# schmeing/ReSeq

Hardware: AMD Instinct MI355X
Metric: simulated read-pairs/sec (2x150 bp) (higher is better)
Workload: dtype f64

## Files before the change

### reseq_amd/csrc/rsq_kernels.h

```cpp
#pragma once
#include "rsq_core.h"
#include "rsq_variants.h"

namespace rsq {

struct Chain {
    uint32_t kind;
    uint32_t id;
    uint32_t seg;
    uint32_t len;
    uint32_t c1, c2;
    uint32_t first_chunk;
    uint32_t initial_dom;
    uint16_t *out;
    uint32_t chunk_lo = 0, in_state = 0;
};

struct ChainAcc {
    const uint64_t *words;
    uint32_t kind, len;
    uint64_t word_off;
    const uint8_t *codes;
    RSQ_HD uint32_t operator()(uint32_t pos) const {
        if (kind == 0) return ref_base(words, word_off, pos);
// ... 959 lines not shown
template <>
struct WordPtr<RSQ_LDS char *> {
    using type = RSQ_LDS uint32_t *;
};
#endif
template <class P>
struct WordSinkT : TextOps<WordSinkT<P>> {
    P p;
    uint64_t acc;
    uint32_t pending, lead, n;
    RSQ_HD explicit WordSinkT(P dst) : p(dst), acc(0), pending(0), lead((4u - ((uint32_t)(uintptr_t)dst & 3u)) & 3u), n(0) {}
    RSQ_HD void push(uint32_t bytes, uint32_t count) {
        acc |= (uint64_t)bytes << (8u * pending);
        pending += count;
        n += count;
        while (lead && pending) {
            *p = (char)(acc & 0xFFu);
            p += 1;
            acc >>= 8;
            --pending;
            --lead;
        }
        if (!lead && pending >= 4u) {
            *reinterpret_cast<typename WordPtr<P>::type>(p) = (uint32_t)acc;
            p += 4;
            acc >>= 32;
            pending -= 4u;
        }
    }
    RSQ_HD void ch(char c) { push((uint8_t)c, 1u); }
    RSQ_HD void bytes(uint32_t word, uint32_t count) { push(count < 4u ? word & ((1u << (8u * count)) - 1u) : word, count); }
    RSQ_HD void finish() {
        while (pending) {
            *p = (char)(acc & 0xFFu);
            p += 1;
            acc >>= 8;
            --pending;
        }
    }
};

RSQ_HD uint32_t digits_u32(uint32_t v) {
    uint32_t n = 1;
    while (v >= 10u) {
        v /= 10u;
        ++n;
    }
    return n;
}
RSQ_HD uint32_t digits_u64(uint64_t v) {
    if (v <= 0xFFFFFFFFull) return digits_u32((uint32_t)v);
    uint32_t n = 1;
    while (v >= 10) {
        v /= 10;
        ++n;
    }
    return n;
}


template <class Sink>
RSQ_HD void format_header(const DevSim &S, const NameTable &names, bool has_f, const Fragment &f, uint64_t adapter_only_number, const ReadMeta &m, const WordColumn &ops, Sink &t,
                          bool has_fv, const FragmentVar &fv) {
    t.ch('@');
    t.str(names.base_identifier, names.base_len);
    if (has_f) {
        const uint32_t end = has_fv ? fv.end : f.start + f.len;
        t.num(f.block);
        t.ch('_');
        t.num(f.number);
        if (1u < S.num_alleles) {
            t.str("_allele", 7);
            t.num((uint32_t)f.allele);
        }
        t.ch(':');
        t.num(f.strand ? end : f.start + 1u);
        t.ch(':');
        t.str(names.names + names.name_ptr[f.seq], names.name_ptr[f.seq + 1] - names.name_ptr[f.seq]);
        t.ch(':');
        t.num(f.strand ? f.start + 1u : end);
    } else {
        t.ch('0');
        t.ch('_');
        t.num(adapter_only_number);
        t.str(":0:Adapter:0", 12);
    }
    t.ch(':');
    t.num((uint32_t)S.tiles[m.tile_id]);
    t.str(":1337:1337 ", 11);
    cigar_replay(ops, m, t);
    t.str(" E", 2);
    t.num((uint32_t)m.num_errors);
    t.ch('\n');
}
template <class Sink>
RSQ_HD void format_header(const DevSim &S, const NameTable &names, const Fragment *f, uint64_t adapter_only_number, const ReadMeta &m, const WordColumn &ops, Sink &t,
                          const FragmentVar *fv = nullptr) {
    format_header(S, names, f != nullptr, f ? *f : Fragment{}, adapter_only_number, m, ops, t, fv != nullptr, fv ? *fv : FragmentVar{});
}
RSQ_HD uint32_t base_letters(uint32_t codes) {
#if defined(__HIP_DEVICE_COMPILE__)
    return __builtin_amdgcn_perm(0x4E4E4E4Eu, 0x54474341u, codes);
#else
    uint32_t out = 0;
    for (uint32_t k = 0; k < 4u; ++k) {
        const uint32_t b = (codes >> (8u * k)) & 0xFFu;
        out |= (uint32_t)("ACGTN"[b < 4u ? b : 4u]) << (8u * k);
    }
    return out;
#endif
}
template <class Sink>
RSQ_HD void format_line_part(const WordColumn &row, uint32_t read_len, bool is_qual, uint32_t first_word, uint32_t n_words, bool with_end, Sink &t) {
    const uint32_t all_words = (read_len + 3u) >> 2, end_word = first_word + n_words < all_words ? first_word + n_words : all_words;
    constexpr uint32_t kAhead = 10u;
    for (uint32_t i = first_word; i < end_word; i += kAhead) {
        uint32_t w[kAhead];
#pragma unroll
        for (uint32_t k = 0; k < kAhead; ++k) w[k] = i + k < end_word ? row.at(i + k) : 0u;
#pragma unroll
        for (uint32_t k = 0; k < kAhead; ++k) {
            const uint32_t at = 4u * (i + k);
            if (i + k >= end_word) break;
            const uint32_t left = read_len - at, text = is_qual ? w[k] : base_letters(w[k]);
            if (left >= 4u) t.push(text, 4u);
            else t.push(text & ((1u << (8u * left)) - 1u), left);
        }
    }
    if (with_end) {
        if (is_qual) t.push('\n', 1u);
        else t.push('\n' | ('+' << 8) | ('\n' << 16), 3u);
    }
}
template <class Sink>
RSQ_HD void format_line(const WordColumn &row, uint32_t read_len, bool is_qual, Sink &t) {
    format_line_part(row, read_len, is_qual, 0u, (read_len + 3u) >> 2, true, t);
}
template <class P>
RSQ_HD uint32_t format_record(const DevSim &S, const NameTable &names, bool has_f, const Fragment &f, uint64_t adapter_only_number, const ReadMeta &m, const WordColumn &seq,
                              const WordColumn &qual, const WordColumn &ops, P dst, bool has_fv, const FragmentVar &fv) {
    WordSinkT<P> t(dst);
    format_header(S, names, has_f, f, adapter_only_number, m, ops, t, has_fv, fv);
    format_line(seq, m.read_len, false, t);
    format_line(qual, m.read_len, true, t);
    t.finish();
    return t.n;
}
template <class P>
RSQ_HD uint32_t format_record(const DevSim &S, const NameTable &names, const Fragment *f, uint64_t adapter_only_number, const ReadMeta &m, const WordColumn &seq,
                              const WordColumn &qual, const WordColumn &ops, P dst, const FragmentVar *fv = nullptr) {
    return format_record(S, names, f != nullptr, f ? *f : Fragment{}, adapter_only_number, m, seq, qual, ops, dst, fv != nullptr, fv ? *fv : FragmentVar{});
}

RSQ_HD uint32_t record_size(const DevSim &S, const NameTable &names, bool has_f, const Fragment &f, uint64_t adapter_only_number, const ReadMeta &m, bool has_fv, const FragmentVar &fv) {
    uint32_t n = 1u + names.base_len;
    if (has_f) {
        const uint32_t end = has_fv ? fv.end : f.start + f.len;
        if (1u < S.num_alleles) n += 7u + digits_u64(f.allele);
        n += digits_u64(f.block) + 1u + digits_u64(f.number) + 1u + digits_u64(f.strand ? end : f.start + 1u) + 1u +
             (names.name_ptr[f.seq + 1] - names.name_ptr[f.seq]) + 1u + digits_u64(f.strand ? f.start + 1u : end);
    } else n += 2u + digits_u64(adapter_only_number) + 12u;
    n += 1u + digits_u64(S.tiles[m.tile_id]) + 11u + m.cigar_chars + 2u + digits_u64(m.num_errors) + 1u;
    return n + 2u * m.read_len + 4u;
}
RSQ_HD uint32_t record_size(const DevSim &S, const NameTable &names, const Fragment *f, uint64_t adapter_only_number, const ReadMeta &m, const FragmentVar *fv = nullptr) {
    return record_size(S, names, f != nullptr, f ? *f : Fragment{}, adapter_only_number, m, fv != nullptr, fv ? *fv : FragmentVar{});
}

struct ReadOut {
    WordColumn seq, qual, ops;
    uint32_t cur_word, cur_index;
    uint32_t seq_word, qual_word, n_put;
    RSQ_HD void put(uint32_t pos, uint32_t base, uint32_t qual_char) {
        const uint32_t sh = (pos & 3u) * 8u;
        seq_word |= base << sh;
        qual_word |= qual_char << sh;
        n_put = pos + 1u;
        if ((pos & 3u) == 3u) {
            seq.at(pos >> 2) = seq_word;
            qual.at(pos >> 2) = qual_word;
            seq_word = qual_word = 0;
        }
    }
    RSQ_HD void op(uint32_t it, uint32_t code) {
        const uint32_t wi = it >> 4;
        if (wi != cur_index) {
            ops.at(cur_index) = cur_word;
            cur_word = 0;
            cur_index = wi;
        }
        cur_word |= code << ((it & 15u) * 2u);
    }
    RSQ_HD void finish() {
        ops.at(cur_index) = cur_word;
        if (n_put & 3u) {
            seq.at(n_put >> 2) = seq_word;
            qual.at(n_put >> 2) = qual_word;
        }
    }
};
RSQ_HD ReadOut make_read_out(const WordColumn &seq, const WordColumn &qual, const WordColumn &ops) { return ReadOut{seq, qual, ops, 0u, 0u, 0u, 0u, 0u}; }

struct RawLayout {
    uint32_t *seq, *qual;
    uint32_t *ops;
    ReadMeta *meta;
    uint64_t pitch;
    uint64_t *templates;
    uint32_t template_words;
    const uint32_t *order;
    RSQ_HD uint64_t item_of(uint64_t row) const { return order ? order[row] : row; }
    RSQ_HD WordColumn seq_of(uint64_t r) const { return WordColumn{seq + r, pitch}; }
    RSQ_HD WordColumn qual_of(uint64_t r) const { return WordColumn{qual + r, pitch}; }
    RSQ_HD WordColumn ops_of(uint64_t r) const { return WordColumn{ops + r, pitch}; }
    RSQ_HD ReadOut out_of(uint64_t r) const { return make_read_out(seq_of(r), qual_of(r), ops_of(r)); }
};

struct FragmentSrc {
    const uint64_t *words;
    uint64_t word_off;
    uint32_t first;
    uint32_t len;
    bool reverse;
    const uint16_t *sys_;
    const uint64_t *converted;
    const uint32_t *gc_prefix;
    mutable uint32_t held_word = 0xFFFFFFFFu, held_sys = 0xFFFFFFFFu;
    mutable uint64_t word = 0, sys4 = 0;
    RSQ_HD uint64_t template_word(const uint64_t *from, uint32_t index) const {
        if (index != held_word) {
            held_word = index;
            word = from[index];
        }
        return word;
    }
    RSQ_HD uint32_t org_len() const { return len; }
    RSQ_HD uint32_t ref(uint32_t k) const {
        const uint32_t pos = reverse ? first - 1u - k : first + k, b = (uint32_t)(template_word(words + word_off, pos >> 5) >> ((pos & 31u) * 2u)) & 3u;
        return reverse ? 3u - b : b;
    }
    RSQ_HD uint32_t base(uint32_t k) const { return converted ? (uint32_t)(template_word(converted, k >> 5) >> ((k & 31u) * 2u)) & 3u : ref(k); }
    RSQ_HD uint32_t sys_base(uint32_t k) const {
        if ((k >> 2) != held_sys) {
            held_sys = k >> 2;
#if defined(__HIP_DEVICE_COMPILE__)
            sys4 = *reinterpret_cast<const uint64_t __attribute__((aligned(2))) *>(sys_ + (k & ~3u));
#else
            memcpy(&sys4, sys_ + (k & ~3u), 8);
#endif
        }
        return (uint32_t)(sys4 >> ((k & 3u) * 16u)) & 0xFFFFu;
    }
    RSQ_HD uint32_t sys_deleted(uint32_t k) const { return sys_base(k); }
    RSQ_HD void totals(uint32_t n, uint32_t &gc, uint32_t &rate_sum) const {
        if (!converted && !gc_prefix) return template_totals_loop(*this, n, gc, rate_sum);
        if (converted) gc += ref_gc_count(converted, 0, 0, n);
        else gc += reverse ? ref_gc_count_prefix(words, gc_prefix, word_off, first - n, first) : ref_gc_count_prefix(words, gc_prefix, word_off, first, first + n);
        rate_sum += rate_total(n);
    }
    RSQ_HD uint32_t rate_total(uint32_t n) const {
        struct __attribute__((packed, aligned(2))) Eight {
            uint64_t a, b;
        };
        uint32_t sum = 0;
        for (uint32_t k = 0; k < n; k += 8u) {
            Eight e;
#if defined(__HIP_DEVICE_COMPILE__)
            e = *reinterpret_cast<const Eight *>(sys_ + k);
#else
            memcpy(&e, sys_ + k, 16);
#endif
            const uint32_t left = n - k;
            if (left < 8u) {
                if (left <= 4u) {
                    e.b = 0;
                    if (left < 4u) e.a &= (1ull << (16u * left)) - 1ull;
                } else e.b &= (1ull << (16u * (left - 4u))) - 1ull;
            }
            const uint64_t kHigh = 0x00FF00FF00FF00FFull, kAdd = 0x0001000100010001ull;
            sum += (uint32_t)((((e.a >> 8) & kHigh) * kAdd) >> 48) + (uint32_t)((((e.b >> 8) & kHigh) * kAdd) >> 48);
        }
        return sum;
    }
};

struct MethView {
    const uint32_t *first, *second;
    const double *rate;
    uint32_t n, stride;
    RSQ_HD double rate_of(int32_t region) const { return rate[(size_t)region * stride]; }
};
RSQ_HD MethView meth_view(const DevSim &S, uint32_t seq, uint32_t allele = 0) {
    const uint32_t off = S.meth_ptr[seq];
    return MethView{S.meth_first + off, S.meth_second + off, S.meth_rate + (size_t)off * S.num_alleles + allele, S.meth_ptr[seq + 1] - off, S.num_alleles};
}
RSQ_HD uint32_t meth_start_index(const MethView &m, uint32_t pos) {
    uint32_t lo = 0, hi = m.n;
    while (lo < hi) {
        const uint32_t mid = (lo + hi) >> 1;
        if (m.second[mid] <= pos) lo = mid + 1;
        else hi = mid;
    }
    return lo;
}
constexpr uint32_t kTemplateWordsMax = 64;
struct MethDraws {
    uint64_t seed;
    uint32_t c0, c1, c2, c3base, have;
    Words w;
    RSQ_HD double uniform(uint32_t k) {
        if (have != (k >> 2)) {
            w = philox(seed, c0, c1, c2, c3base | (k >> 2));
            have = k >> 2;
        }
        const uint32_t j = k & 3u;
        return u32_to_unit(j == 0u ? w.w0 : (j == 1u ? w.w1 : (j == 2u ? w.w2 : w.w3)));
    }
};
RSQ_HD void ct_convert_run(uint64_t *tmpl, uint32_t t, uint32_t n, double rate, MethDraws &d) {
    const uint32_t end = t + n;
    for (uint32_t w = t >> 5; (w << 5) < end; ++w) {
        const uint32_t lo = t > (w << 5) ? t - (w << 5) : 0u, hi = end - (w << 5) < 32u ? end - (w << 5) : 32u;
        uint64_t cs = tmpl[w] & ~(tmpl[w] >> 1) & 0x5555555555555555ull;
        cs &= (hi == 32u ? ~0ull : (1ull << (2u * hi)) - 1ull) & ~((1ull << (2u * lo)) - 1ull);
        while (cs) {
#if defined(__HIP_DEVICE_COMPILE__)
            const uint32_t bit = (uint32_t)__ffsll((long long)cs) - 1u;
#else
            const uint32_t bit = (uint32_t)__builtin_ctzll(cs);
#endif
            cs &= cs - 1ull;
            if (d.uniform((w << 5) + (bit >> 1)) < rate) tmpl[w] |= (uint64_t)3u << bit;
        }
    }
}
template <bool REV>
struct MethSide {
    const MethView &m;
    const VarView *r;
    uint32_t allele;
    int32_t lowest;
    RSQ_HD int64_t coord(uint32_t pos) const { return REV ? -(int64_t)pos : (int64_t)pos; }
    RSQ_HD int64_t entry(int32_t i) const { return REV ? 1 - (int64_t)m.second[i] : (int64_t)m.first[i]; }
    RSQ_HD int64_t exit(int32_t i) const { return REV ? 1 - (int64_t)m.first[i] : (int64_t)m.second[i]; }
    RSQ_HD bool region(int32_t i) const { return REV ? i >= lowest : i < (int32_t)m.n; }
    RSQ_HD bool variant(int32_t j) const { return r && (REV ? j >= 0 : j < (int32_t)r->n); }
    RSQ_HD static int32_t next(int32_t i) { return REV ? i - 1 : i + 1; }
    RSQ_HD int64_t at(int32_t j) const { return coord(r->v[j].pos); }
    RSQ_HD uint32_t len(int32_t j) const { return r->v[j].len; }
    RSQ_HD bool mine(int32_t j) const { return r->in_allele(r->v[j], allele); }
    RSQ_HD int32_t first_region(uint32_t pos) const {
        if (!REV) return (int32_t)meth_start_index(m, pos);
        uint32_t lo = 0, hi = m.n;
        while (lo < hi) {
            const uint32_t mid = (lo + hi) >> 1;
            if (m.first[mid] <= pos) lo = mid + 1;
            else hi = mid;
        }
        return (int32_t)lo - 1;
    }
};
template <bool REV>
RSQ_HD void methylation_walk(uint64_t *tmpl, uint32_t length, const MethView &m, const VarView *r, uint32_t allele, uint32_t start_pos, VarStart from, MethDraws &d) {
    const MethSide<REV> side{m, r, allele, r ? 0 : 1};
    int64_t x = side.coord(start_pos);
    uint16_t t = 0;
    int32_t region = side.first_region(start_pos), var = r ? from.first_variant_id : -1;
    uint32_t left = 0;
    if (side.variant(var) && side.at(var) == x && side.len(var) > 1u && side.mine(var)) left = side.len(var) - from.start_variant_pos;
// ... 958 lines not shown
#endif
        RSQ_LDS float *img = fill_stage_image<MASK>(S, lds_image, qbase);
#if defined(RSQ_TRACE_FILL)
        if (threadIdx.x == 0) trace[1] = wall_clock64();
#endif
        const uint32_t lane = threadIdx.x & 63u;
        const uint32_t n_mine = job.rec_count[seg];
        const uint32_t *index = job.rec_index + (seg ? job.rec_count[0] : 0u);
        for (;;) {
            uint32_t chunk = 0;
            if (lane == 0) chunk = atomicAdd(&chunk_counters[seg], 1u);
            chunk = __shfl(chunk, 0, 64);
            const uint64_t first = (uint64_t)chunk * 64u;
            if (first >= n_mine) break;
            const bool active = first + lane < n_mine;
            const uint32_t i = active ? index[first + lane] : 0u;
            fill_record_chunk<MASK, false, PACKED>(S, job, img, qbase, seg, 0u, i, i, active, raw);
#if defined(RSQ_TRACE_FILL)
            if (lane == 0) atomicAdd(reinterpret_cast<unsigned long long *>(trace + 3), 1ull);
#endif
        }
#if defined(RSQ_TRACE_FILL)
        if (lane == 0) atomicMax(reinterpret_cast<unsigned long long *>(trace + 2), (unsigned long long)wall_clock64());
#endif
    }
}
template <uint32_t MASK, bool BINNED = false, bool PACKED = false>
__global__ void __launch_bounds__(kFillBlockWalk) k_fill_records(DevSim S, RecordJob job, RawLayout raw, uint32_t *chunk_counters, FillBins bins) {
    fill_records_body<MASK, BINNED, PACKED>(S, job, raw, chunk_counters, bins);
}
#if !defined(RSQ_SPEC)
struct FragmentRange {
    uint32_t lo[2], hi[2];
};
__global__ void k_fragment_range(const uint8_t *segs, const uint32_t *frag_len, uint64_t n, FragmentRange range, uint32_t *first_bad) {
    const uint64_t i = (uint64_t)blockIdx.x * blockDim.x + threadIdx.x;
    if (i >= n) return;
    const uint32_t seg = segs[i] ? 1u : 0u, fl = frag_len[i];
    if (fl < range.lo[seg] || fl >= range.hi[seg]) atomicMin(first_bad, (uint32_t)i);
}
__global__ void k_record_flags(const uint8_t *segs, uint64_t n, uint32_t *flags) {
    const uint64_t i = (uint64_t)blockIdx.x * blockDim.x + threadIdx.x;
    if (i < n) flags[i] = segs[i] ? 1u : 0u;
}
__global__ void k_record_partition(const uint8_t *segs, uint64_t n, const uint64_t *ones_before, uint32_t *rec_index, uint32_t *rec_count) {
    const uint64_t i = (uint64_t)blockIdx.x * blockDim.x + threadIdx.x;
    const uint32_t n1 = (uint32_t)ones_before[n], n0 = (uint32_t)n - n1;
    if (i == 0) {
        rec_count[0] = n0;
        rec_count[1] = n1;
    }
    if (i >= n) return;
    const uint32_t before = (uint32_t)ones_before[i];
    if (segs[i]) rec_index[n0 + before] = (uint32_t)i;
    else rec_index[(uint32_t)i - before] = (uint32_t)i;
}

__global__ void __launch_bounds__(256) k_methylation_templates(DevSim S, const Fragment *frags, uint64_t n_pairs, RawLayout raw) {
    const uint64_t r = (uint64_t)blockIdx.x * blockDim.x + threadIdx.x;
    if (r >= 2u * n_pairs) return;
    const uint32_t seg = r >= n_pairs ? 1u : 0u;
    convert_template(S, frags[r - seg * n_pairs], seg, raw.templates + r * raw.template_words, raw.template_words);
}

__global__ void __launch_bounds__(256) k_variant_templates(DevSim S, const Fragment *frags, const FragmentVar *fvars, uint64_t n_pairs, RawLayout raw) {
    const uint64_t r = (uint64_t)blockIdx.x * blockDim.x + threadIdx.x;
    if (r >= 2u * n_pairs) return;
    const uint32_t seg = r >= n_pairs ? 1u : 0u;
    const uint64_t pair = r - seg * n_pairs;
    variant_template(S, frags[pair], fvars[pair], seg, raw.templates + r * raw.template_words, raw.template_words);
}

#endif
#endif

#if RSQ_DEVICE_BUILD && !defined(RSQ_SPEC)
#ifndef RSQ_FORMAT_RECORDS
#define RSQ_FORMAT_RECORDS 16
#endif
constexpr uint32_t kFormatRecords = RSQ_FORMAT_RECORDS, kFormatLdsMax = 16u * 1024u, kFormatLdsMin = 1024u;
RSQ_HD uint32_t format_lds_bytes(uint64_t record_bytes) {
    const uint64_t want = (kFormatRecords * record_bytes + 16u + 127u) & ~(uint64_t)127u;
    return (uint32_t)(want < kFormatLdsMin ? kFormatLdsMin : want > kFormatLdsMax ? kFormatLdsMax : want);
}
__global__ void __launch_bounds__(256) k_max_size(const uint32_t *sizes, uint64_t n, uint32_t *longest) {
    uint32_t m = 0;
    for (uint64_t i = (uint64_t)blockIdx.x * blockDim.x + threadIdx.x; i < n; i += (uint64_t)gridDim.x * blockDim.x) m = max(m, sizes[i]);
    for (uint32_t d = 32; d; d >>= 1) m = max(m, (uint32_t)__shfl_xor((int)m, (int)d, 64));
    if ((threadIdx.x & 63u) == 0 && m) atomicMax(longest, m);
}
template <bool PERM>
__global__ void __launch_bounds__(64) k_format_write(DevSim S, NameTable names, const Fragment *frags, uint64_t n_pairs, uint64_t adapter_only_first, RawLayout raw,
                                                    const uint64_t *offsets0, const uint64_t *offsets1, char *dst0, char *dst1, uint64_t cap0, uint64_t cap1,
                                                    const FragmentVar *fvars, const uint32_t *perm, uint32_t lds_bytes) {
    extern __shared__ __attribute__((aligned(16))) char s_text[];
    const uint32_t lane = threadIdx.x, seg = blockIdx.y, rec = lane & (kFormatRecords - 1u), part = lane / kFormatRecords;
    constexpr uint32_t kLineParts = 32u / kFormatRecords;
    const bool is_qual = part >= kLineParts;
    const uint32_t sub = part % kLineParts;
    const uint64_t first = (uint64_t)blockIdx.x * kFormatRecords;
    if (first >= n_pairs) return;
    const uint64_t *offsets = seg ? offsets1 : offsets0;
    char *dst = seg ? dst1 : dst0;
    if (offsets[n_pairs] > (seg ? cap1 : cap0)) return;
    const uint64_t last = first + kFormatRecords < n_pairs ? first + kFormatRecords : n_pairs;
    const uint64_t row = first + rec;
    const bool active = row < last;
    const uint64_t pair = PERM ? (active ? perm[row] : 0u) : row;
    const uint64_t g_begin = PERM ? (active ? offsets[pair] : 0u) : offsets[first], g_end = PERM ? (active ? offsets[pair + 1u] : 0u) : offsets[last];
    const uint32_t skew = (uint32_t)((uint64_t)(uintptr_t)(dst + g_begin) & 15u), bytes = (uint32_t)(g_end - g_begin);
    const uint32_t kSlot = (lds_bytes / kFormatRecords) & ~15u;
    const bool through_lds = PERM ? __all(skew + bytes <= kSlot) != 0 : skew + bytes <= lds_bytes;
    ReadMeta m;
    Fragment f;
    FragmentVar fv;
    uint64_t r = 0;
    if (active) {
        r = (uint64_t)seg * n_pairs + row;
        m = raw.meta[r];
        if (frags) f = frags[pair];
        if (frags && fvars) fv = fvars[pair];
    }
    const WordColumn seq = raw.seq_of(r), qual = raw.qual_of(r), ops = raw.ops_of(r);
    const uint64_t ao_number = adapter_only_first + pair + 1u;
    if (!through_lds) {
        if (active && part == 0u) format_record(S, names, frags != nullptr, f, ao_number, m, seq, qual, ops, dst + offsets[pair], frags && fvars, fv);
        return;
    }
    const uint32_t slot_at = PERM ? rec * kSlot : 0u;
    if (active) {
        RSQ_LDS char *rec_text = (RSQ_LDS char *)s_text + slot_at + skew + (PERM ? 0u : (uint32_t)(offsets[pair] - g_begin));
        const uint32_t header = (uint32_t)(offsets[pair + 1u] - offsets[pair]) - 2u * m.read_len - 4u;
        const uint32_t all_words = (m.read_len + 3u) >> 2, per = (all_words + kLineParts - 1u) / kLineParts;
        const uint32_t first_word = sub * per, line_at = header + (is_qual ? m.read_len + 3u : 0u);
        const uint32_t part_at = part == 0u ? 0u : line_at + (4u * first_word < m.read_len ? 4u * first_word : m.read_len);
        WordSinkT<RSQ_LDS char *> t(rec_text + part_at);
        if (part == 0u) format_header(S, names, frags != nullptr, f, ao_number, m, ops, t, frags && fvars, fv);
        format_line_part(is_qual ? qual : seq, m.read_len, is_qual, first_word, per, sub == kLineParts - 1u, t);
        t.finish();
    }
    __syncthreads();
    const uint32_t lo = skew, hi = skew + bytes;
    char *g_chunk0 = dst + g_begin - skew;
    const char *s_from = s_text + slot_at;
    for (uint32_t c = (PERM ? part : lane) * 16u; c < hi; c += (PERM ? 64u / kFormatRecords : 64u) * 16u) {
        if (c >= lo && c + 16u <= hi) {
            *reinterpret_cast<uint4 *>(g_chunk0 + c) = *reinterpret_cast<const uint4 *>(s_from + c);
        } else {
            for (uint32_t b = c < lo ? lo : c; b < c + 16u && b < hi; ++b) g_chunk0[b] = s_from[b];
        }
    }
}

#endif

}
```

### reseq_amd/csrc/rsq_sim.hip

```cpp
#include <hip/hip_runtime.h>
#include <fcntl.h>
#include <sys/mman.h>
#include <sys/stat.h>
#include <math.h>
#include <string.h>
#include <unistd.h>

#include <algorithm>
#include <atomic>
#include <chrono>
#include <map>
#include <thread>
#include <memory>
#include <string>
#include <utility>
#include <vector>

#include "../../include/reseq_amd.h"
#include "rsq_deflate.h"
#include "rsq_fasta.h"
#include "rsq_pack.h"
#include "rsq_spec.h"
#include "rsq_textio.h"

// ... 484 lines not shown
    HIP_CHECK(hipMemsetAsync(s.cur->fill_counters.as<uint32_t>(), 0, 8, st));
    hipFunction_t spec = spec_kernel(s, SpecKind::kReads, MASK, VAR, BINNED);
    s.timers["fill_reads"].start(st);
    if (spec) {
        uint32_t *sizes = s.cur->sizes.as<uint32_t>(), *counters = s.cur->fill_counters.as<uint32_t>();
        RawLayout raw_arg = raw;
        void *args[] = {&s.dev, &s.names, &frags, &n_pairs, &adapter_first, &raw_arg, &sizes, &counters, &fvars, &bins};
        spec_allow_lds(spec, lds_bytes);
        HIP_CHECK(hipModuleLaunchKernel(spec, blocks, 1, 1, kBlock, 1, 1, (unsigned)lds_bytes, st, args, nullptr));
    } else
        hipLaunchKernelGGL((k_fill_reads<MASK, VAR, BINNED>), dim3(blocks), dim3(kBlock), lds_bytes, st, s.dev, s.names, frags, n_pairs, adapter_first, raw, s.cur->sizes.as<uint32_t>(),
                           s.cur->fill_counters.as<uint32_t>(), fvars, bins);
    s.timers["fill_reads"].stop(st);
    HIP_CHECK(hipGetLastError());
    return bins.perm;
}
template <uint32_t MASK, bool VAR = false>
static const uint32_t *launch_fill_mask(rsq_sim &s, const Fragment *frags, uint64_t n_pairs, uint64_t adapter_first, const RawLayout &raw, hipStream_t st, const FragmentVar *fvars = nullptr) {
    if constexpr (MASK != 0)
        if (fill_is_binned(s)) return launch_fill_kernel<MASK, VAR, true>(s, frags, n_pairs, adapter_first, raw, st, fvars);
    return launch_fill_kernel<MASK, VAR, false>(s, frags, n_pairs, adapter_first, raw, st, fvars);
}
template <uint32_t MASK, bool BINNED, bool PACKED>
static const uint32_t *launch_records_kernel(rsq_sim &s, const RecordJob &job, const uint8_t *seg_dev, uint64_t n, const RawLayout &raw, hipStream_t st) {
    FillBins bins{};
    if (BINNED)
        bins = build_fill_bins(s, n, 2 * s.dev.n_tiles, st, [&](uint16_t *keys, uint32_t *hist) {
            hipLaunchKernelGGL(k_record_tiles, dim3(cdiv(n, kBinBlock)), dim3(kBinBlock), 0, st, s.dev, seg_dev, job.first_index, n, keys, hist);
        });
    const size_t lds_bytes = fill_lds_bytes(s, MASK != 0, BINNED, &k_fill_records<MASK, BINNED, PACKED>);
    const FillShape shape = fill_shape(s, lds_bytes, n, 1, kFillBlockWalk);
    const uint32_t blocks = shape.blocks;
#if defined(RSQ_TRACE_FILL)
    s.cur->fill_counters.reserve(16 + 32 * (size_t)blocks);
    HIP_CHECK(hipMemsetAsync(s.cur->fill_counters.as<uint32_t>(), 0, 16 + 32 * (size_t)blocks, st));
#else
    s.cur->fill_counters.reserve(8);
    HIP_CHECK(hipMemsetAsync(s.cur->fill_counters.as<uint32_t>(), 0, 8, st));
#endif
    hipFunction_t spec = spec_kernel(s, SpecKind::kRecords, MASK, PACKED, BINNED);
    s.timers["fill_reads"].start(st);
    if (spec) {
        uint32_t *counters = s.cur->fill_counters.as<uint32_t>();
        RecordJob job_arg = job;
        RawLayout raw_arg = raw;
        void *args[] = {&s.dev, &job_arg, &raw_arg, &counters, &bins};
        spec_allow_lds(spec, lds_bytes);
        HIP_CHECK(hipModuleLaunchKernel(spec, blocks, 1, 1, shape.threads, 1, 1, (unsigned)lds_bytes, st, args, nullptr));
    } else
        hipLaunchKernelGGL((k_fill_records<MASK, BINNED, PACKED>), dim3(blocks), dim3(shape.threads), lds_bytes, st, s.dev, job, raw, s.cur->fill_counters.as<uint32_t>(), bins);
    s.timers["fill_reads"].stop(st);
#if defined(RSQ_TRACE_FILL)
    {
        std::vector<uint64_t> t(2 + 4 * (size_t)blocks);
        HIP_CHECK(hipMemcpyAsync(t.data(), s.cur->fill_counters.as<uint64_t>(), t.size() * 8, hipMemcpyDeviceToHost, st));
        HIP_CHECK(hipStreamSynchronize(st));
        uint64_t first = ~0ull, last_start = 0, last_end = 0, stage = 0, run = 0;
        for (uint32_t b = 0; b < blocks; ++b) {
            first = std::min(first, t[2 + 4 * b]);
            last_start = std::max(last_start, t[2 + 4 * b]);
            last_end = std::max(last_end, t[4 + 4 * b]);
            stage += t[3 + 4 * b] - t[2 + 4 * b];
            run += t[4 + 4 * b] - t[3 + 4 * b];
        }
        if (getenv("RSQ_TRACE_WORKGROUPS")) {
            std::string line;
            for (uint32_t b = 0; b < blocks; ++b) {
                line += " " + std::to_string(b) + ":" + std::to_string((t[2 + 4 * b] - first) / 100) + "+" + std::to_string((t[4 + 4 * b] - t[2 + 4 * b]) / 100) + "/" + std::to_string(t[5 + 4 * b]);
            }
            fprintf(stderr, "trace_fill workgroup:start+duration(us)/chunks:%s\n", line.c_str());
        }
        fprintf(stderr, "trace_fill: %u workgroups of %u threads, %llu items: last start %.1f us after the first, last end %.1f us; image staged in %.1f us, chunks %.1f us (means; 100 MHz clock)\n", blocks,
                shape.threads, (unsigned long long)n, (last_start - first) / 100.0, (last_end - first) / 100.0, stage / 100.0 / blocks, run / 100.0 / blocks);
    }
#endif
    HIP_CHECK(hipGetLastError());
    return bins.perm;
}
template <uint32_t MASK>
static const uint32_t *launch_records_mask(rsq_sim &s, const RecordJob &job, const uint8_t *seg_dev, uint64_t n, const RawLayout &raw, hipStream_t st) {
    if constexpr (MASK != 0)
        if (fill_is_binned(s)) return job.codes ? launch_records_kernel<MASK, true, true>(s, job, seg_dev, n, raw, st) : launch_records_kernel<MASK, true, false>(s, job, seg_dev, n, raw, st);
    return job.codes ? launch_records_kernel<MASK, false, true>(s, job, seg_dev, n, raw, st) : launch_records_kernel<MASK, false, false>(s, job, seg_dev, n, raw, st);
}
static const uint32_t *launch_fill_reads(rsq_sim &s, const Fragment *frags, uint64_t n_pairs, uint64_t adapter_first, const RawLayout &raw, hipStream_t st,
                              const FragmentVar *fvars = nullptr) {
    const uint32_t mask = effective_fill_mask(s.dev.lds.mask, s.force_fill_mode);
    const bool var = frags && s.has_variants;
#define RSQ_FILL_CASE(Q)                                                                       \
    if (mask == Q) {                                                                                  \
        if (var) return launch_fill_mask<Q, true>(s, frags, n_pairs, adapter_first, raw, st, fvars);  \
        return launch_fill_mask<Q>(s, frags, n_pairs, adapter_first, raw, st);                        \
    }
    RSQ_FILL_CASE(0u)
    RSQ_FILL_CASE(kQualityQuads[0])
    RSQ_FILL_CASE(kQualityQuads[1])
    RSQ_FILL_CASE(kQualityQuads[2])
    RSQ_FILL_CASE(kQualityQuads[3])
    RSQ_FILL_CASE(kQualityQuads[4])
    static_assert(sizeof(kQualityQuads) == 5 * sizeof(uint32_t), "one case per entry");
#undef RSQ_FILL_CASE
    throw Error("no k_fill_reads instantiation for " + std::to_string(mask) + " quads");
}
static const uint32_t *launch_fill_records(rsq_sim &s, const RecordJob &job, const uint8_t *seg_dev, uint64_t n, const RawLayout &raw, hipStream_t st) {
    const uint32_t mask = effective_fill_mask(s.dev.lds.mask, s.force_fill_mode);
#define RSQ_REC_CASE(Q) \
    if (mask == Q) return launch_records_mask<Q>(s, job, seg_dev, n, raw, st);
    RSQ_REC_CASE(0u)
    RSQ_REC_CASE(kQualityQuads[0])
    RSQ_REC_CASE(kQualityQuads[1])
    RSQ_REC_CASE(kQualityQuads[2])
    RSQ_REC_CASE(kQualityQuads[3])
    RSQ_REC_CASE(kQualityQuads[4])
#undef RSQ_REC_CASE
    throw Error("no k_fill_records instantiation for " + std::to_string(mask) + " quads");
}

struct ReadsDone {
    RawLayout raw;
    const uint32_t *row_order;
};
static ReadsDone reads_stage(rsq_sim &s, const Fragment *frags, uint64_t n_pairs, uint64_t adapter_first, hipStream_t st, const FragmentVar *fvars) {
    RawLayout raw = raw_layout(s, 2 * n_pairs);
    s.cur->sizes.reserve(2 * n_pairs * 4 + 16);
    if (frags && s.dev.meth_ptr && !fvars) {
        s.cur->templates.reserve(2 * n_pairs * s.template_words * 8 + 16);
        raw.templates = s.cur->templates.as<uint64_t>();
        raw.template_words = s.template_words;
        hipLaunchKernelGGL(k_methylation_templates, dim3(cdiv(2 * n_pairs, 256)), dim3(256), 0, st, s.dev, frags, n_pairs, raw);
        HIP_CHECK(hipGetLastError());
    }
    if (frags && fvars) {
        s.cur->templates.reserve(2 * n_pairs * s.template_words * 8 + 16);
        raw.templates = s.cur->templates.as<uint64_t>();
        raw.template_words = s.template_words;
        s.timers["variant_templates"].start(st);
        hipLaunchKernelGGL(k_variant_templates, dim3(cdiv(2 * n_pairs, 256)), dim3(256), 0, st, s.dev, frags, fvars, n_pairs, raw);
        s.timers["variant_templates"].stop(st);
        HIP_CHECK(hipGetLastError());
    }
    const uint32_t *row_order = launch_fill_reads(s, frags, n_pairs, adapter_first, raw, st, fvars);
    return ReadsDone{raw, row_order};
}
static void text_stage(rsq_sim &s, const Fragment *frags, uint64_t n_pairs, uint64_t adapter_first, const ReadsDone &rd, char *r1, size_t r1_cap, char *r2, size_t r2_cap,
                       uint32_t part, hipStream_t st, const FragmentVar *fvars) {
    rsq_sim::Workspace &w = *s.cur;
    w.off_r1.reserve((n_pairs + 1) * 8);
    w.off_r2.reserve((n_pairs + 1) * 8);
    uint64_t *totals = s.totals.as<uint64_t>();
    s.timers["scan"].start(st);
    exclusive_scan(s, w.sizes.as<uint32_t>(), n_pairs, w.off_r1.as<uint64_t>(), st, totals + 2 * part, totals + 2 * (part + 1));
    exclusive_scan(s, w.sizes.as<uint32_t>() + n_pairs, n_pairs, w.off_r2.as<uint64_t>(), st, totals + 2 * part + 1, totals + 2 * (part + 1) + 1);
    s.timers["scan"].stop(st);
    const dim3 grid(cdiv(n_pairs, kFormatRecords), 2), block(64);
    const uint32_t lds = rd.row_order ? std::min(kFormatLdsMax, format_lds_bytes(s.format_record_bytes) + 16u * kFormatRecords) : format_lds_bytes(s.format_record_bytes);
    hipLaunchKernelGGL(k_max_size, dim3(std::min<uint64_t>(1024, cdiv(2 * n_pairs, 256))), dim3(256), 0, st, w.sizes.as<uint32_t>(), 2 * n_pairs, s.longest_record.as<uint32_t>());
    s.timers["format_write"].start(st);
    if (rd.row_order)
        hipLaunchKernelGGL(k_format_write<true>, grid, block, lds, st, s.dev, s.names, frags, n_pairs, adapter_first, rd.raw, w.off_r1.as<uint64_t>(), w.off_r2.as<uint64_t>(), r1, r2,
                           (uint64_t)(r1 ? r1_cap : 0), (uint64_t)(r2 ? r2_cap : 0), fvars, rd.row_order, lds);
    else
        hipLaunchKernelGGL(k_format_write<false>, grid, block, lds, st, s.dev, s.names, frags, n_pairs, adapter_first, rd.raw, w.off_r1.as<uint64_t>(), w.off_r2.as<uint64_t>(), r1, r2,
                           (uint64_t)(r1 ? r1_cap : 0), (uint64_t)(r2 ? r2_cap : 0), fvars, (const uint32_t *)nullptr, lds);
    s.timers["format_write"].stop(st);
    HIP_CHECK(hipGetLastError());
}
static void reset_call_timers(rsq_sim &s) {
    for (auto &t : s.timers) t.second.reset();
}
static int finish_call(rsq_sim &s, uint32_t parts, bool with_variants, char *r1, size_t r1_cap, size_t *r1_len, char *r2, size_t r2_cap, size_t *r2_len, hipStream_t text_stream) {
    s.mailbox[4] = 0;
    if (with_variants) HIP_CHECK(hipMemcpyAsync(&s.mailbox[4], s.dev.walk_error, 4, hipMemcpyDeviceToHost, text_stream));
    HIP_CHECK(hipMemcpyAsync(&s.mailbox[2], s.totals.as<uint64_t>() + 2 * parts, 16, hipMemcpyDeviceToHost, text_stream));
    HIP_CHECK(hipMemcpyAsync(&s.mailbox[5], s.longest_record.as<uint32_t>(), 4, hipMemcpyDeviceToHost, text_stream));
    HIP_CHECK(hipStreamSynchronize(text_stream));
    *r1_len = s.mailbox[2];
    *r2_len = s.mailbox[3];
    if ((uint32_t)s.mailbox[4]) {
        HIP_CHECK(hipMemsetAsync(s.dev.walk_error, 0, 4, text_stream));
        HIP_CHECK(hipStreamSynchronize(text_stream));
        g_last_error = kWalkErrorMessage;
        return RSQ_EINVAL;
    }
    if (*r1_len > r1_cap || *r2_len > r2_cap || !r1 || !r2) {
        g_last_error = "output buffers too small: need " + std::to_string(*r1_len) + " and " + std::to_string(*r2_len) + " bytes";
        return RSQ_ENOSPC;
    }
    return RSQ_OK;
}
static void begin_totals(rsq_sim &s, uint32_t parts, hipStream_t st) {
    s.totals.reserve((size_t)(parts + 1) * 16 + 16);
    s.longest_record.reserve(8);
    HIP_CHECK(hipMemsetAsync(s.totals.as<uint64_t>(), 0, 16, st));
    HIP_CHECK(hipMemsetAsync(s.longest_record.as<uint32_t>(), 0, 4, st));
}

static int adapter_only_pairs(rsq_sim &s, uint64_t n_pairs, uint64_t adapter_first, char *r1, size_t r1_cap, size_t *r1_len, char *r2, size_t r2_cap, size_t *r2_len, hipStream_t st) {
    *r1_len = *r2_len = 0;
    if (!n_pairs) return RSQ_OK;
    reset_call_timers(s);
    s.cur = &s.ws[0];
    begin_totals(s, 1, st);
    const ReadsDone rd = reads_stage(s, nullptr, n_pairs, adapter_first, st, nullptr);
    text_stage(s, nullptr, n_pairs, adapter_first, rd, r1, r1_cap, r2, r2_cap, 0, st, nullptr);
    return finish_call(s, 1, false, r1, r1_cap, r1_len, r2, r2_cap, r2_len, st);
}

struct SieveRun {
    uint32_t block_lo = 0, block_hi = 0;
    uint64_t n_slots = 0, cand_cap = 0, hit_cap = 0, total = 0, n_cands = 0;
    uint32_t n_hits = 0;
    const SlotInfo *slot_table = nullptr;
};
static void sieve_attempt(rsq_sim &s, SieveRun &r, int attempt, uint64_t *mail, hipStream_t st) {
    rsq_sim::Workspace &w = *s.cur;
    const int vm = s.variants_mode;
    if (r.cand_cap >= (1ull << 32)) throw Error("more than 2^32 sieve candidates in one call: use smaller block ranges");
    w.cands.reserve(r.cand_cap * sizeof(SieveCand));
    w.pairs_of.reserve(r.cand_cap * 4 + 16);
    w.pair_off.reserve((r.cand_cap + 1) * 8);
    if (vm) w.hits.reserve(r.hit_cap * sizeof(SieveHit));
    else w.cell_info.reserve(r.cand_cap * 4 + 16);
    HIP_CHECK(hipMemsetAsync(w.hit_count.as<uint32_t>(), 0, 4, st));
    s.timers["sieve"].start(st);
    const uint32_t block_lo = r.block_lo, block_hi = r.block_hi;
    const uint64_t n_slots = r.n_slots, cand_cap = r.cand_cap;
    const dim3 ggrid(cdiv(n_slots, kSieveBlock)), gblock(kSieveBlock);
    if (!attempt) {
        if (2 == vm) {
            w.slot_table.reserve(n_slots * sizeof(SlotInfo) + 16);
            s.timers["slot_table"].start(st);
            hipLaunchKernelGGL(k_slot_table, dim3(block_hi - block_lo), dim3(256), 0, st, s.dev, block_lo, w.slot_table.as<SlotInfo>());
            s.timers["slot_table"].stop(st);
            r.slot_table = w.slot_table.as<SlotInfo>();
        }
        s.timers["sieve_screen"].start(st);
        if (2 == vm)
            hipLaunchKernelGGL((k_sieve_gaps<2, false>), ggrid, gblock, 0, st, s.dev, block_lo, block_hi, (uint32_t)n_slots, w.counts.as<uint32_t>(), (const uint64_t *)nullptr,
                               (SieveCand *)nullptr, cand_cap, r.slot_table);
        else
            hipLaunchKernelGGL((k_sieve_gaps<0, false>), ggrid, gblock, 0, st, s.dev, block_lo, block_hi, (uint32_t)n_slots, w.counts.as<uint32_t>(), (const uint64_t *)nullptr,
                               (SieveCand *)nullptr, cand_cap, r.slot_table);
        s.timers["sieve_screen"].stop(st);
        exclusive_scan(s, w.counts.as<uint32_t>(), n_slots, w.offsets.as<uint64_t>(), st);
    }
    const SlotInfo *slot_table = r.slot_table;
    if (2 == vm)
        hipLaunchKernelGGL((k_sieve_gaps<2, true>), ggrid, gblock, 0, st, s.dev, block_lo, block_hi, (uint32_t)n_slots, (uint32_t *)nullptr, w.offsets.as<uint64_t>(),
                           w.cands.as<SieveCand>(), cand_cap, slot_table);
    else
        hipLaunchKernelGGL((k_sieve_gaps<0, true>), ggrid, gblock, 0, st, s.dev, block_lo, block_hi, (uint32_t)n_slots, (uint32_t *)nullptr, w.offsets.as<uint64_t>(),
                           w.cands.as<SieveCand>(), cand_cap, slot_table);
    const dim3 fgrid(cdiv(cand_cap, kSieveBlock)), fblock(kSieveBlock);
#define RSQ_FINISH(VM, CAP)                                                                                                                                   \
    hipLaunchKernelGGL((k_sieve_finish<VM, CAP>), fgrid, fblock, 0, st, s.dev, block_lo, block_hi, (uint32_t)n_slots, w.offsets.as<uint64_t>(), w.cands.as<SieveCand>(),  \
                       cand_cap, w.pairs_of.as<uint32_t>(), w.hits.as<SieveHit>(), (uint32_t)std::min<uint64_t>(r.hit_cap, 0xFFFFFFFFull), w.hit_count.as<uint32_t>(), slot_table, \
                       w.cell_info.as<uint32_t>())
    if (2 == vm && s.num_alleles <= 8) RSQ_FINISH(2, 8);
    else if (2 == vm) RSQ_FINISH(2, kMaxDevAlleles);
    else if (1 == vm) RSQ_FINISH(1, 8);
    else RSQ_FINISH(0, 1);
#undef RSQ_FINISH
    s.timers["sieve"].stop(st);
    HIP_CHECK(hipGetLastError());
    exclusive_scan(s, w.pairs_of.as<uint32_t>(), cand_cap, w.pair_off.as<uint64_t>(), st);
    mail[1] = 0;
    HIP_CHECK(hipMemcpyAsync(&mail[0], w.pair_off.as<uint64_t>() + cand_cap, 8, hipMemcpyDeviceToHost, st));
    HIP_CHECK(hipMemcpyAsync(&mail[1], w.hit_count.as<uint32_t>(), 4, hipMemcpyDeviceToHost, st));
    HIP_CHECK(hipMemcpyAsync(&mail[5], w.offsets.as<uint64_t>() + n_slots, 8, hipMemcpyDeviceToHost, st));
}
static bool sieve_launch(rsq_sim &s, SieveRun &r, uint32_t block_lo, uint32_t block_hi, uint64_t *mail, hipStream_t st) {
    rsq_sim::Workspace &w = *s.cur;
    const int vm = s.variants_mode;
    r = SieveRun{};
    r.block_lo = block_lo;
    r.block_hi = block_hi;
    r.n_slots = (uint64_t)(block_hi - block_lo) * kBlockSize;
    if (2 == vm && block_hi > block_lo) {
        uint32_t ptr[2];
        HIP_CHECK(hipMemcpy(&ptr[0], s.dev.block_extra_ptr + block_lo, 4, hipMemcpyDeviceToHost));
        HIP_CHECK(hipMemcpy(&ptr[1], s.dev.block_extra_ptr + block_hi, 4, hipMemcpyDeviceToHost));
        r.n_slots += ptr[1] - ptr[0];
    }
    if (!r.n_slots) return false;
    if (r.n_slots >= (1ull << 32) - kSieveBlock)
        throw Error("block range too large for one call: at most " + std::to_string(((1ull << 32) - kSieveBlock) / kBlockSize - 1) + " blocks");
    w.counts.reserve(r.n_slots * 4 + 16);
    w.offsets.reserve((r.n_slots + 1) * 8);
    w.hit_count.reserve(8);
    const double expected_cands = s.expected_passing * (double)r.n_slots;
    r.cand_cap = std::max<uint64_t>(w.cands.bytes() / sizeof(SieveCand), (uint64_t)(expected_cands + 6.0 * sqrt(expected_cands + 1.0)) + 65536);
    r.hit_cap = std::max<uint64_t>(w.hits.bytes() / sizeof(SieveHit), 0 == vm ? r.cand_cap : r.cand_cap + r.cand_cap / 4);
    sieve_attempt(s, r, 0, mail, st);
    return true;
}
static void sieve_collect(rsq_sim &s, SieveRun &r, uint64_t *mail, hipStream_t st) {
    for (int attempt = 0;; ++attempt) {
        HIP_CHECK(hipStreamSynchronize(st));
        r.total = mail[0];
        r.n_hits = (uint32_t)mail[1];
        r.n_cands = mail[5];
        if (r.n_cands <= r.cand_cap && r.n_hits <= r.hit_cap) return;
        if (attempt >= 2) throw Error("sieve lists overflowed three times");
        const double grow = r.n_cands > r.cand_cap ? (double)r.n_cands / (double)r.cand_cap : 1.0;
        if (r.n_hits > r.hit_cap || grow > 1.0) r.hit_cap = std::max<uint64_t>(r.hit_cap, (uint64_t)((double)r.n_hits * grow * 1.25) + 65536);
        r.cand_cap = std::max(r.cand_cap, r.n_cands + 65536);
        sieve_attempt(s, r, attempt + 1, mail, st);
    }
}
static void sieve_emit(rsq_sim &s, const SieveRun &r, hipStream_t st) {
    rsq_sim::Workspace &w = *s.cur;
    w.frags.reserve(r.total * sizeof(Fragment) + 16);
    s.timers["sieve_emit"].start(st);
    if (2 == s.variants_mode) {
        w.fvars.reserve(r.total * sizeof(FragmentVar) + 16);
        hipLaunchKernelGGL(k_sieve_emit<2>, dim3(cdiv(r.n_hits, 256)), dim3(256), 0, st, s.dev, r.block_lo, r.block_hi, w.hits.as<SieveHit>(), r.n_hits, w.offsets.as<uint64_t>(),
// ... 1900 lines not shown
```

Measured before the change: 225.9 million.

## Format FASTQ text directly to global memory with word-aligned funnel-shift stores

For the unordered case, the LDS-staged k_format_write kernel is replaced by a new k_format_text kernel. In it, each lane of a 64-thread block writes one read's sequence or quality line straight to global memory. Lines go out as aligned 32-bit words built with alignbyte funnel shifts, and the header is written by the sequence lane. This removes the shared-memory staging and the barrier-separated copy-out, but global writes become per-lane strided rather than coalesced 16-byte chunks. The ordered path still uses the old kernel, and format_text_lds_bytes is defined but never used.

```diff
diff --git a/reseq_amd/csrc/rsq_kernels.h b/reseq_amd/csrc/rsq_kernels.h
--- a/reseq_amd/csrc/rsq_kernels.h
+++ b/reseq_amd/csrc/rsq_kernels.h
@@ -1135,6 +1135,55 @@
     return format_record(S, names, f != nullptr, f ? *f : Fragment{}, adapter_only_number, m, seq, qual, ops, dst, fv != nullptr, fv ? *fv : FragmentVar{});
 }
 
+RSQ_HD uint32_t funnel_bytes(uint32_t hi, uint32_t lo, uint32_t shift) {
+#if defined(__HIP_DEVICE_COMPILE__)
+    return __builtin_amdgcn_alignbyte(hi, lo, shift);
+#else
+    return (uint32_t)((((uint64_t)hi << 32) | lo) >> (8u * shift));
+#endif
+}
+template <class P>
+RSQ_HD void format_line_words(const WordColumn &row, uint32_t read_len, bool is_qual, P line) {
+    using WordP = typename WordPtr<P>::type;
+    const uint32_t total = read_len + (is_qual ? 1u : 3u), full = read_len >> 2, rest = read_len & 3u;
+    const uint64_t end = is_qual ? (uint64_t)'\n' : (uint64_t)('\n' | '+' << 8 | '\n' << 16);
+    const uint32_t last_raw = rest ? row.at(full) : 0u, last_text = is_qual ? last_raw : base_letters(last_raw);
+    const uint64_t tail = (rest ? (uint64_t)(last_text & ((1u << (8u * rest)) - 1u)) : 0u) | end << (8u * rest);
+    if (total < 8u) {
+        const uint32_t first_raw = full ? row.at(0) : 0u;
+        const uint64_t text = full ? (is_qual ? first_raw : base_letters(first_raw)) | tail << 32 : tail;
+        for (uint32_t b = 0; b < total; ++b) line[b] = (char)(text >> (8u * b));
+        return;
+    }
+    const uint32_t head = (4u - ((uint32_t)(uintptr_t)line & 3u)) & 3u;
+    const uint32_t first_raw = row.at(0), first_text = is_qual ? first_raw : base_letters(first_raw);
+    uint32_t prev = first_text;
+    P out = line + head;
+    constexpr uint32_t kAhead = 40u;
+    for (uint32_t i = 1; i < full; i += kAhead) {
+        uint32_t w[kAhead];
+#pragma unroll
+        for (uint32_t k = 0; k < kAhead; ++k) w[k] = i + k < full ? row.at(i + k) : 0u;
+#pragma unroll
+        for (uint32_t k = 0; k < kAhead; ++k) {
+            if (i + k >= full) break;
+            const uint32_t text = is_qual ? w[k] : base_letters(w[k]);
+            *reinterpret_cast<WordP>(out + 4u * (i + k - 1u)) = funnel_bytes(text, prev, head);
+            prev = text;
+        }
+    }
+    for (uint32_t b = 0; b < head; ++b) line[b] = (char)(first_text >> (8u * b));
+#pragma unroll
+    for (uint32_t j = 0; j < 3u; ++j) {
+        const uint32_t text = j == 0u ? (uint32_t)tail : j == 1u ? (uint32_t)(tail >> 32) : 0u, v = funnel_bytes(text, prev, head);
+        const uint32_t at = head + 4u * (full + j - 1u);
+        prev = text;
+        if (at + 4u <= total) *reinterpret_cast<WordP>(line + at) = v;
+        else
+            for (uint32_t b = 0; at + b < total; ++b) line[at + b] = (char)(v >> (8u * b));
+    }
+}
+
 RSQ_HD uint32_t record_size(const DevSim &S, const NameTable &names, bool has_f, const Fragment &f, uint64_t adapter_only_number, const ReadMeta &m, bool has_fv, const FragmentVar &fv) {
     uint32_t n = 1u + names.base_len;
     if (has_f) {
@@ -1198,6 +1247,30 @@
     RSQ_HD WordColumn ops_of(uint64_t r) const { return WordColumn{ops + r, pitch}; }
     RSQ_HD ReadOut out_of(uint64_t r) const { return make_read_out(seq_of(r), qual_of(r), ops_of(r)); }
 };
+
+constexpr uint32_t kTextGroup = 32u;
+template <class P>
+RSQ_HD void format_group_lane(uint32_t lane, const DevSim &S, const NameTable &names, const Fragment *frags, const FragmentVar *fvars, uint64_t adapter_only_first,
+                              const RawLayout &raw, uint64_t n_pairs, uint32_t seg, const uint64_t *offsets, uint64_t first, uint64_t last, P image) {
+    const bool is_qual = lane >= kTextGroup;
+    const uint64_t pair = first + lane % kTextGroup;
+    if (pair >= last) return;
+    const uint64_t r = (uint64_t)seg * n_pairs + pair;
+    const ReadMeta m = raw.meta[r];
+    const uint64_t at = offsets[pair] - offsets[first];
+    const uint32_t header = (uint32_t)(offsets[pair + 1u] - offsets[pair]) - 2u * m.read_len - 4u;
+    P text = image + at;
+    Fragment f{};
+    FragmentVar fv{};
+    if (!is_qual && frags) f = frags[pair];
+    if (!is_qual && frags && fvars) fv = fvars[pair];
+    format_line_words(is_qual ? raw.qual_of(r) : raw.seq_of(r), m.read_len, is_qual, text + header + (is_qual ? m.read_len + 3u : 0u));
+    if (!is_qual) {
+        WordSinkT<P> t(text);
+        format_header(S, names, frags != nullptr, f, adapter_only_first + pair + 1u, m, raw.ops_of(r), t, frags && fvars, fv);
+        t.finish();
+    }
+}
 
 struct FragmentSrc {
     const uint64_t *words;
@@ -2462,6 +2535,24 @@
     }
 }
 
-#endif
-
-}
+constexpr uint32_t kTextLdsMax = 32u * 1024u;
+RSQ_HD uint32_t format_text_lds_bytes(uint64_t record_bytes) {
+    const uint64_t want = (kTextGroup * record_bytes + 16u + 127u) & ~(uint64_t)127u;
+    return (uint32_t)(want < kFormatLdsMin ? kFormatLdsMin : want > kTextLdsMax ? kTextLdsMax : want);
+}
+__global__ void __launch_bounds__(64) k_format_text(DevSim S, NameTable names, const Fragment *frags, uint64_t n_pairs, uint64_t adapter_only_first, RawLayout raw,
+                                                   const uint64_t *offsets0, const uint64_t *offsets1, char *dst0, char *dst1, uint64_t cap0, uint64_t cap1,
+                                                   const FragmentVar *fvars) {
+    const uint32_t lane = threadIdx.x, seg = blockIdx.y;
+    const uint64_t first = (uint64_t)blockIdx.x * kTextGroup;
+    if (first >= n_pairs) return;
+    const uint64_t *offsets = seg ? offsets1 : offsets0;
+    char *dst = seg ? dst1 : dst0;
+    if (offsets[n_pairs] > (seg ? cap1 : cap0)) return;
+    const uint64_t last = first + kTextGroup < n_pairs ? first + kTextGroup : n_pairs;
+    format_group_lane(lane, S, names, frags, fvars, adapter_only_first, raw, n_pairs, seg, offsets, first, last, dst + offsets[first]);
+}
+
+#endif
+
+}
diff --git a/reseq_amd/csrc/rsq_sim.hip b/reseq_amd/csrc/rsq_sim.hip
--- a/reseq_amd/csrc/rsq_sim.hip
+++ b/reseq_amd/csrc/rsq_sim.hip
@@ -660,16 +660,17 @@
     exclusive_scan(s, w.sizes.as<uint32_t>(), n_pairs, w.off_r1.as<uint64_t>(), st, totals + 2 * part, totals + 2 * (part + 1));
     exclusive_scan(s, w.sizes.as<uint32_t>() + n_pairs, n_pairs, w.off_r2.as<uint64_t>(), st, totals + 2 * part + 1, totals + 2 * (part + 1) + 1);
     s.timers["scan"].stop(st);
-    const dim3 grid(cdiv(n_pairs, kFormatRecords), 2), block(64);
-    const uint32_t lds = rd.row_order ? std::min(kFormatLdsMax, format_lds_bytes(s.format_record_bytes) + 16u * kFormatRecords) : format_lds_bytes(s.format_record_bytes);
+    const dim3 block(64);
     hipLaunchKernelGGL(k_max_size, dim3(std::min<uint64_t>(1024, cdiv(2 * n_pairs, 256))), dim3(256), 0, st, w.sizes.as<uint32_t>(), 2 * n_pairs, s.longest_record.as<uint32_t>());
     s.timers["format_write"].start(st);
-    if (rd.row_order)
-        hipLaunchKernelGGL(k_format_write<true>, grid, block, lds, st, s.dev, s.names, frags, n_pairs, adapter_first, rd.raw, w.off_r1.as<uint64_t>(), w.off_r2.as<uint64_t>(), r1, r2,
-                           (uint64_t)(r1 ? r1_cap : 0), (uint64_t)(r2 ? r2_cap : 0), fvars, rd.row_order, lds);
-    else
-        hipLaunchKernelGGL(k_format_write<false>, grid, block, lds, st, s.dev, s.names, frags, n_pairs, adapter_first, rd.raw, w.off_r1.as<uint64_t>(), w.off_r2.as<uint64_t>(), r1, r2,
-                           (uint64_t)(r1 ? r1_cap : 0), (uint64_t)(r2 ? r2_cap : 0), fvars, (const uint32_t *)nullptr, lds);
+    if (rd.row_order) {
+        const uint32_t lds = std::min(kFormatLdsMax, format_lds_bytes(s.format_record_bytes) + 16u * kFormatRecords);
+        hipLaunchKernelGGL(k_format_write<true>, dim3(cdiv(n_pairs, kFormatRecords), 2), block, lds, st, s.dev, s.names, frags, n_pairs, adapter_first, rd.raw, w.off_r1.as<uint64_t>(),
+                           w.off_r2.as<uint64_t>(), r1, r2, (uint64_t)(r1 ? r1_cap : 0), (uint64_t)(r2 ? r2_cap : 0), fvars, rd.row_order, lds);
+    } else {
+        hipLaunchKernelGGL(k_format_text, dim3(cdiv(n_pairs, kTextGroup), 2), block, 0, st, s.dev, s.names, frags, n_pairs, adapter_first, rd.raw, w.off_r1.as<uint64_t>(),
+                           w.off_r2.as<uint64_t>(), r1, r2, (uint64_t)(r1 ? r1_cap : 0), (uint64_t)(r2 ? r2_cap : 0), fvars);
+    }
     s.timers["format_write"].stop(st);
     HIP_CHECK(hipGetLastError());
 }
```

After: 190.5 million (median of 2 runs). -15.7%, worse.
